# alexisvannson/GraphNet_Classifier

Measured on AMD Instinct MI355X. Metric: edges aggregated/sec (GraphNet forward), higher is better.
Workload: dtype f32; 1 GPU; c3: 1M nodes / 10M edges (6250 graphs x 160 nodes x 1600 edges), D=64, 2 GN blocks; graphs=6250, nodes=1000000, edges=10000000, n_blocks=2, width=64, step=CSR build + GraphNet.forward, inputs resident in HBM

## Files before the change

### graphnet_classifier_amd/csrc/mlp_device.h

```cpp
#pragma once
#include "gnc_common.h"

namespace gnc_mlp {

typedef float f32x16 __attribute__((ext_vector_type(16)));
typedef float f32x4 __attribute__((ext_vector_type(4)));

constexpr int KC = 64;
constexpr int LDSW = 68;
constexpr int RPW = 32;

__device__ __forceinline__ f32x16 mfma(float a, float b, f32x16 c) {
  return __builtin_amdgcn_mfma_f32_32x32x2f32(a, b, c, 0, 0, 0);
}

__device__ __forceinline__ void wave_lds_fence() {
  asm volatile("s_waitcnt lgkmcnt(0)" ::: "memory");
}

__device__ __forceinline__ float activate(float x, int act, float p) {
  switch (act) {
    case GNC_ACT_RELU: return x < 0.f ? 0.f : x;
    case GNC_ACT_IDENTITY: return x;
    case GNC_ACT_TANH: return tanhf(x);
    case GNC_ACT_SIGMOID: return 1.f / (1.f + expf(-x));
    case GNC_ACT_SILU: return x / (1.f + expf(-x));
    case GNC_ACT_GELU: return 0.5f * x * (1.f + erff(x * 0.70710678118654752440f));
    case GNC_ACT_LEAKY_RELU: return x < 0.f ? x * p : x;
    case GNC_ACT_ELU: return x > 0.f ? x : p * expm1f(x);
    default: return x;
  }
}

template <int T>
__device__ __forceinline__ void activate_tiles(f32x16 (&acc)[T], int act, float p) {
  if (act == GNC_ACT_RELU) {
#pragma unroll
    for (int t = 0; t < T; ++t)
#pragma unroll
      for (int r = 0; r < 16; ++r) acc[t][r] = acc[t][r] < 0.f ? 0.f : acc[t][r];
  } else {
#pragma unroll
    for (int t = 0; t < T; ++t)
#pragma unroll
      for (int r = 0; r < 16; ++r) acc[t][r] = activate(acc[t][r], act, p);
  }
}

__device__ __forceinline__ constexpr int feat_of(int t, int r, int h) { return 32 * t + (r & 3) + 8 * (r >> 2) + 4 * h; }

__device__ __forceinline__ f32x4 load4_guarded(const float* p, int col, int limit, bool vec_ok) {
  f32x4 v = {0.f, 0.f, 0.f, 0.f};
  if (vec_ok && col + 4 <= limit) {
    v = *reinterpret_cast<const f32x4*>(p);
  } else {
    if (col + 0 < limit) v.x = p[0];
    if (col + 1 < limit) v.y = p[1];
    if (col + 2 < limit) v.z = p[2];
    if (col + 3 < limit) v.w = p[3];
  }
  return v;
}

template <int TROWS, int NT>
__device__ __forceinline__ void stage_weights(float* wbuf, const float* __restrict__ W, int ldw, int out_dim,
                                              int kbase, int klimit, int ncol4, bool vec_ok, int tid) {
  constexpr int RPP = NT / 16;
  static_assert(TROWS % RPP == 0, "weight rows must be a multiple of the rows staged per pass");
  const int c4 = tid & 15;
  const int r0 = tid >> 4;
  if (c4 < ncol4) {
#pragma unroll
    for (int p = 0; p < TROWS / RPP; ++p) {
      const int n = p * RPP + r0;
      f32x4 v = {0.f, 0.f, 0.f, 0.f};
      if (n < out_dim) v = load4_guarded(W + (int64_t)n * ldw + kbase + c4 * 4, kbase + c4 * 4, klimit, vec_ok);
      *reinterpret_cast<f32x4*>(wbuf + n * LDSW + c4 * 4) = v;
    }
  }
}

template <int NT>
__device__ __forceinline__ void stage_params(float* pbuf, const gnc_mlp_desc_t& d, int pstride, int tid) {
  const int L = d.num_linear;
  const int out_dim = d.out_dim[L - 1];
  for (int idx = tid; idx < (L + 2) * pstride; idx += NT) {
    const int l = idx / pstride, n = idx - l * pstride;
    float v = 0.f;
    if (l < L) {
      if (d.bias[l] && n < d.out_dim[l]) v = d.bias[l][n];
    } else if (d.ln_gamma && n < out_dim) {
      v = (l == L) ? d.ln_gamma[n] : (d.ln_beta ? d.ln_beta[n] : 0.f);
    }
    pbuf[idx] = v;
  }
}

template <int T>
__device__ __forceinline__ void init_bias(f32x16 (&acc)[T], const float* pb, int h) {
#pragma unroll
  for (int t = 0; t < T; ++t)
#pragma unroll
    for (int q = 0; q < 4; ++q) {
      const f32x4 b = *reinterpret_cast<const f32x4*>(pb + 32 * t + 8 * q + 4 * h);
      acc[t][4 * q + 0] = b.x; acc[t][4 * q + 1] = b.y; acc[t][4 * q + 2] = b.z; acc[t][4 * q + 3] = b.w;
    }
}

template <int T>
__device__ __forceinline__ void mma_chunk_from_lds(f32x16 (&acc)[T], const float* abuf, const float* wbuf, int kc8,
                                                   int i, int h) {
#pragma unroll(T >= 4 ? 1 : 2)
  for (int g = 0; g < kc8; ++g) {
    const f32x4 b = *reinterpret_cast<const f32x4*>(abuf + i * LDSW + 8 * g + 4 * h);
#pragma unroll
    for (int t = 0; t < T; ++t) {
      const f32x4 a = *reinterpret_cast<const f32x4*>(wbuf + (32 * t + i) * LDSW + 8 * g + 4 * h);
      acc[t] = mfma(a.x, b.x, acc[t]);
      acc[t] = mfma(a.y, b.y, acc[t]);
      acc[t] = mfma(a.z, b.z, acc[t]);
      acc[t] = mfma(a.w, b.w, acc[t]);
    }
  }
}

template <int T>
__device__ __forceinline__ void add_rows_from_lds(f32x16 (&acc)[T], const float* abuf, int t0, int i, int h) {
#pragma unroll
  for (int tt = 0; tt < 2; ++tt) {
#pragma unroll
    for (int t = 0; t < T; ++t) {
      if (t == t0 + tt) {
#pragma unroll
        for (int q = 0; q < 4; ++q) {
          const f32x4 v = *reinterpret_cast<const f32x4*>(abuf + i * LDSW + 32 * tt + 8 * q + 4 * h);
          acc[t][4 * q + 0] += v.x; acc[t][4 * q + 1] += v.y; acc[t][4 * q + 2] += v.z; acc[t][4 * q + 3] += v.w;
        }
      }
    }
  }
}

template <int TI, int TO>
__device__ __forceinline__ void mma_chunk_from_regs(f32x16 (&dst)[TO], const f32x16 (&src)[TI], const float* wbuf,
                                                    int c, int in_dim, int i, int h) {
#pragma unroll
  for (int g = 0; g < 8; ++g) {
    const int ts = 2 * c + (g >> 2);
    if (ts < TI && c * KC + g * 8 < in_dim) {
      const int q = g & 3;
#pragma unroll
      for (int t = 0; t < TO; ++t) {
        const f32x4 a = *reinterpret_cast<const f32x4*>(wbuf + (32 * t + i) * LDSW + 8 * g + 4 * h);
        dst[t] = mfma(a.x, src[ts < TI ? ts : 0][4 * q + 0], dst[t]);
        dst[t] = mfma(a.y, src[ts < TI ? ts : 0][4 * q + 1], dst[t]);
        dst[t] = mfma(a.z, src[ts < TI ? ts : 0][4 * q + 2], dst[t]);
        dst[t] = mfma(a.w, src[ts < TI ? ts : 0][4 * q + 3], dst[t]);
      }
      if constexpr (TO >= 4) __builtin_amdgcn_sched_barrier(0);
    }
  }
}

typedef __bf16 bf16x8 __attribute__((ext_vector_type(8)));
typedef float f32x8 __attribute__((ext_vector_type(8)));

constexpr int SLDW = 72;
constexpr int SPLANE = 64 * SLDW;
constexpr int SCH = 3 * SPLANE / 2;

// ... 766 lines not shown
#pragma unroll
    for (int q = 0; q < 4; ++q) {
      f32x4 v = {o[TA][4 * q + 0], o[TA][4 * q + 1], o[TA][4 * q + 2], o[TA][4 * q + 3]};
      *reinterpret_cast<f32x4*>(abuf + i * LDSW + 32 * TT + 8 * q + 4 * h) = v;
    }
  }
}
template <int T, int T0>
__device__ __forceinline__ void chunk_to_lds(const f32x16 (&o)[T], float* abuf, int i, int h) {
  one_tile_to_lds<T, T0, 0>(o, abuf, i, h);
  one_tile_to_lds<T, T0 + 1, 1>(o, abuf, i, h);
}

struct SegView {
  const float* ptr;
  const int32_t* index;
  int ld;
  int width;
  uint32_t bytes;
};


struct BwdArgs {
  const float* grad_out;
  int ld_grad_out;
  float* act[GNC_MAX_LINEAR];
  float* dz[GNC_MAX_LINEAR];
  float* dx;
  int ld_dx;
  float* yhat;
  int dx_add_grad_out;
  float* ln_partial;
  const float* gg;
  const int* gg_index;
  int ld_gg;
  int64_t gg_rows;
  float* g_sum;
  int ld_g_sum;
};

__host__ __device__ inline int ldw_of(const gnc_mlp_desc_t& d, int l) { return d.ld_weight[l] ? d.ld_weight[l] : d.in_dim[l]; }

inline bool al16(const void* p) { return (reinterpret_cast<uintptr_t>(p) & 15u) == 0; }

inline int tiles_for(int width) {
  const int t = (width + 31) / 32;
  return t <= 1 ? 1 : t <= 2 ? 2 : t <= 4 ? 4 : 8;
}

int validate_desc(const gnc_mlp_desc_t* d, bool check_ptrs);
int launch_resident_dual(const float* x, int64_t ld_x, int64_t rows, const float* wa, int64_t ld_wa, const float* wb, int64_t ld_wb,
                         int in_dim, int out_dim, float* out_a, float* out_b, int64_t ld_out, hipStream_t stream, bool* launched);
int launch_resident(const gnc_mlp_desc_t& d, int T, bool narrow_out, hipStream_t stream, bool* launched,
                    bool probe_only = false, bool agg_only = false);
int launch_stream(const gnc_mlp_desc_t& d, int T, bool narrow_out, hipStream_t stream, bool* launched,
                  bool probe_only = false);
int launch_stream16(const gnc_mlp_desc_t& d, hipStream_t stream, bool* launched, bool probe_only = false);
int launch_col16(const gnc_mlp_desc_t& d, hipStream_t stream, bool* launched, bool probe_only = false);
int64_t col16_max_rows();
int64_t bwd_col16_max_rows();
bool bwd_col16_supported(const gnc_mlp_desc_t& d);
int bwd_col16_ln_partial_rows(int64_t rows);
int launch_bwd_col16(const gnc_mlp_bwd_desc_t& bd, hipStream_t stream);
bool bwd_col16_persist_supported(const gnc_mlp_desc_t& d);
int bwd_col16_persist_ln_partial_rows(int64_t rows);
int launch_bwd_col16_persist(const gnc_mlp_bwd_desc_t& bd, hipStream_t stream);
bool bwd_stream16_supported(const gnc_mlp_desc_t& d, bool want_dx);
int bwd_stream16_ln_partial_rows(int64_t rows);
int launch_bwd_stream16(const gnc_mlp_desc_t& d, const BwdArgs& b, hipStream_t stream, bool saved = false);

}
```

### graphnet_classifier_amd/csrc/mlp_fused.hip

```cpp
#include <stdlib.h>

#include "mlp_device.h"

using namespace gnc_mlp;

namespace {

constexpr int WAVES = 4;
constexpr int NT = WAVES * 64;
constexpr int RPB = RPW * WAVES;

__device__ __forceinline__ void stage_rows(float* abuf, const gnc_mlp_segment_t& seg, int64_t row0, int64_t rows,
                                           int c0, int ncol4, bool vec_ok, int lane) {
  const int c4 = lane & 15;
  const int rs = lane >> 4;
  if (c4 < ncol4) {
#pragma unroll
    for (int p = 0; p < RPW / 4; ++p) {
      const int j = p * 4 + rs;
      const int64_t r = row0 + j;
      f32x4 v = {0.f, 0.f, 0.f, 0.f};
      if (r < rows) {
        const int64_t tr = seg.index ? (int64_t)seg.index[r] : r;
        if (!seg.index || (uint64_t)tr < (uint64_t)seg.table_rows)
// ... 375 lines not shown
    gnc::set_error("gnc_mlp_operands_in_place_supported: this description runs on a kernel that reads rows of 16-B pieces");
    return GNC_ERR_UNSUPPORTED;
  }
  return GNC_OK;
}

extern "C" int gnc_mlp_edge_features_supported(const gnc_mlp_desc_t* desc) {
  int rc = validate_desc(desc, false);
  if (rc) return rc;
  const auto [T, narrow_out] = tile_class(*desc);
  gnc_mlp_desc_t probe = *desc;
  alignas(16) static float dummy_f[4];
  static int32_t dummy_i[1];
  if (!probe.ef_pos) probe.ef_pos = dummy_f;
  if (!probe.ef_src) probe.ef_src = dummy_i;
  if (!probe.ef_dst) probe.ef_dst = dummy_i;
  bool ok = false;
  {
    gnc_mlp_desc_t plain = *desc;
    plain.ef_pos = nullptr;
    if (!plain.seg[0].ptr) plain.seg[0].ptr = dummy_f;
    bool small = false;
    rc = launch_col16(plain, nullptr, &small, true);
    if (rc) return rc;
    if (!small && desc->rows > 0) {
      rc = launch_resident(probe, T, narrow_out, nullptr, &ok, true);
      if (rc) return rc;
    }
  }
  if (!ok) {
    gnc::set_error("gnc_mlp_edge_features_supported: needs the edge encoder's shape on the weights-resident kernel (one computed "
                   "segment of width 3 = space_dim 2, >= 2 Linear layers of widths 33..64, ReLU, no residual / save_act / agg_out) "
                   "and a batch above the small-batch limit");
    return GNC_ERR_UNSUPPORTED;
  }
  return GNC_OK;
}

extern "C" int gnc_mlp_small_batch_supported(const gnc_mlp_desc_t* desc) {
  int rc = validate_desc(desc, false);
  if (rc) return rc;
  FwdKernel k = FwdKernel::none;
  if (desc->rows > 0) {
    rc = forward_chain(*desc, nullptr, true, &k);
    if (rc) return rc;
  }
  if (k != FwdKernel::col16) {
    gnc::set_error("gnc_mlp_small_batch_supported: not a small-batch description (rows, widths <= 128, ReLU)");
    return GNC_ERR_UNSUPPORTED;
  }
  return GNC_OK;
}

extern "C" int gnc_mlp_forward_f32(const gnc_mlp_desc_t* desc, void* stream_) {
  int rc = validate_desc(desc, true);
  if (rc) return rc;
  if (desc->rows == 0) return GNC_OK;
  hipStream_t stream = (hipStream_t)stream_;
  if (desc->ef_pos) {
    rc = gnc_mlp_edge_features_supported(desc);
    if (rc) return rc;
    const auto [T, narrow_out] = tile_class(*desc);
    bool launched = false;
    rc = launch_resident(*desc, T, narrow_out, stream, &launched);
    if (!rc && !launched) {
      gnc::set_error("gnc_mlp_forward_f32: ef_pos given but the weights-resident kernel did not take the launch");
      rc = GNC_ERR_UNSUPPORTED;
    }
    return rc;
  }
  FwdKernel k;
  return forward_chain(*desc, stream, false, &k);
}
```

### graphnet_classifier_amd/csrc/mlp_resident.hip

```cpp
#include <stdlib.h>

#include "mlp_device.h"

using namespace gnc_mlp;

#ifdef GNC_PHASE_PROBE
__device__ unsigned long long gnc_phase_probe[4096 * 12];
extern "C" int gnc_phase_probe_read(void* dst, size_t bytes) {
  return (int)hipMemcpyFromSymbol(dst, HIP_SYMBOL(gnc_phase_probe), bytes);
}
#define PROBE_BEGIN() unsigned long long pr_acc[8] = {0, 0, 0, 0, 0, 0, 0, 0}, pr_tp, pr_tn; \
  const unsigned long long pr_c0 = __builtin_readcyclecounter(), pr_w0 = wall_clock64()
#define PROBE_TILE() pr_tp = __builtin_readcyclecounter()
#define PROBE(k) do { pr_tn = __builtin_readcyclecounter(); pr_acc[k] += pr_tn - pr_tp; pr_tp = pr_tn; } while (0)
#define PROBE_END() do { if ((threadIdx.x & 63) == 0) {                                                      \
    unsigned long long* o = gnc_phase_probe + (blockIdx.x * (blockDim.x >> 6) + (threadIdx.x >> 6)) * 12;    \
    for (int k = 0; k < 8; ++k) o[k] = pr_acc[k];                                                            \
    o[8] = __builtin_readcyclecounter() - pr_c0; o[9] = wall_clock64() - pr_w0; } } while (0)
#else
#define PROBE_BEGIN() do {} while (0)
#define PROBE_TILE() do {} while (0)
#define PROBE(k) do {} while (0)
#define PROBE_END() do {} while (0)
#endif

namespace {

constexpr int RWAVES = 8;
constexpr int RNT = RWAVES * 64;

template <int HT, int OT, int NMM, int NADD, bool RESREG, bool AGG = false, bool SAVE = false, bool FULL = false, int EF = 0, bool DUAL = false,
          int SPLIT = 0, bool AGGONLY = false>
__global__ __launch_bounds__(RNT) void mlp_resident_kernel(const gnc_mlp_desc_t d, const int num_wtiles,
                                                           const int total_chunks) {
  extern __shared__ __attribute__((aligned(16))) float lds[];
  constexpr int WT = HT > OT ? HT : OT;
  constexpr int CH = WT * 32 * LDSW;
  static_assert(!FULL || OT == 2, "fixed widths: 64 out");
  static_assert(!FULL || NADD == 2 || (NMM == 1 && !RESREG && !AGG && !SAVE && !DUAL), "fixed-width plain stacks");
  constexpr int SEGW = EF != 0 ? 3 : KC;
  constexpr bool W32 = FULL && !SAVE;
  constexpr bool GADD = W32 && NADD == 2;
  static_assert(SPLIT == 0 || (HT == 2 && SPLIT == 1 && NMM == 1 && ((NADD == 2 && RESREG && !DUAL) || (NADD == 0 && !RESREG))) ||
                    (HT == 2 && OT == 2 && SPLIT == 2 && NADD == 0 && !DUAL),
                "split shapes");
  constexpr int nf32 = SPLIT == 1 ? 0 : NMM;
  constexpr bool SPK = !(SPLIT == 1 && NADD == 2 && AGG && !FULL && !SAVE);
  constexpr bool PIPE = SPLIT != 0 && SPK && !DUAL && (FULL || (SPLIT == 2 && NMM == 1) || (SPLIT == 1 && NADD == 0));
  constexpr bool FRONT = GADD && SPLIT == 1 && PIPE;
  constexpr int GPK = FRONT ? 4 : 2;
  __bf16* const wsp = reinterpret_cast<__bf16*>(lds + nf32 * CH);
  auto wsplit = [&](int chunk) -> const __bf16* { return wsp + (chunk - nf32) * 3 * SPLANE; };
  constexpr int PSTRIDE = WT * 32;
  constexpr int NS = NMM + NADD;
  const int tid = threadIdx.x;
  const int lane = tid & 63;
  const int wave = __builtin_amdgcn_readfirstlane(tid >> 6);
  const int i = lane & 31;
  const int h = lane >> 5;
  const int c4 = lane & 15;
  const int rs = lane >> 4;
  const int L = FULL ? 3 : d.num_linear;
  const int out_dim = FULL ? KC : d.out_dim[L - 1];
  const int rows = (int)d.rows;
  float* wres = lds;
  float* pbuf = SPLIT == 0 ? lds + total_chunks * CH : lds + nf32 * CH + (total_chunks - nf32) * SCH;
  float* abuf = pbuf + (L + 2) * PSTRIDE + wave * RPW * LDSW;

  stage_params<RNT>(pbuf, d, PSTRIDE, tid);
  if constexpr (SPLIT != 0) {
    const int ldw0 = ldw_of(d, 0);
    const bool w0v = (ldw0 % 4 == 0) && ((reinterpret_cast<uintptr_t>(d.weight[0]) & 15u) == 0);
    if constexpr (SPLIT == 1) {
      stage_weights_split<RNT>(wsp, d.weight[0], ldw0, d.out_dim[0], d.seg[0].wcol, d.seg[0].wcol + d.seg[0].width,
                               w0v && (d.seg[0].wcol % 4 == 0), tid);
    } else {
#pragma unroll
      for (int s = 0; s < NMM; ++s)
        stage_weights<WT * 32, RNT>(wres + s * CH, d.weight[0], ldw0, d.out_dim[0], d.seg[s].wcol, d.seg[s].wcol + d.seg[s].width, 16,
                                    w0v && (d.seg[s].wcol % 4 == 0), tid);
    }
    if constexpr (DUAL) {
      const int ldw1 = ldw_of(d, 1);
      const bool w1v = (ldw1 % 4 == 0) && ((reinterpret_cast<uintptr_t>(d.weight[1]) & 15u) == 0) && (d.seg[0].wcol % 4 == 0);
      stage_weights_split<RNT>(wsp + 3 * SPLANE, d.weight[1], ldw1, d.out_dim[0], d.seg[0].wcol, d.seg[0].wcol + d.seg[0].width, w1v, tid);
    }
    for (int l = 1; l < L; ++l) {
      const int ldw = ldw_of(d, l);
      const bool wv = (ldw % 4 == 0) && ((reinterpret_cast<uintptr_t>(d.weight[l]) & 15u) == 0);
      stage_weights_split<RNT>(wsp + (NMM + l - 1 - nf32) * 3 * SPLANE, d.weight[l], ldw, d.out_dim[l], 0, d.in_dim[l], wv, tid);
    }
  } else {
    int chunk = 0;
    const int ldw0 = ldw_of(d, 0);
    const bool w0v = (ldw0 % 4 == 0) && ((reinterpret_cast<uintptr_t>(d.weight[0]) & 15u) == 0);
#pragma unroll
    for (int s = 0; s < NMM; ++s, ++chunk)
      stage_weights<WT * 32, RNT>(wres + chunk * CH, d.weight[0], ldw0, d.out_dim[0], d.seg[s].wcol,
                                  d.seg[s].wcol + d.seg[s].width, 16, w0v && (d.seg[s].wcol % 4 == 0), tid);
    for (int l = 1; l < L; ++l) {
      const int ldw = ldw_of(d, l);
      const bool wv = (ldw % 4 == 0) && ((reinterpret_cast<uintptr_t>(d.weight[l]) & 15u) == 0);
      for (int c = 0; c * KC < d.in_dim[l]; ++c, ++chunk)
        stage_weights<WT * 32, RNT>(wres + chunk * CH, d.weight[l], ldw, d.out_dim[l], c * KC, d.in_dim[l], 16, wv, tid);
    }
    if constexpr (DUAL) {
      const int ldw1 = ldw_of(d, 1);
      const bool w1v = (ldw1 % 4 == 0) && ((reinterpret_cast<uintptr_t>(d.weight[1]) & 15u) == 0);
      stage_weights<WT * 32, RNT>(wres + CH, d.weight[1], ldw1, d.out_dim[0], d.seg[0].wcol, d.seg[0].wcol + d.seg[0].width, 16,
                                  w1v && (d.seg[0].wcol % 4 == 0), tid);
    }
  }
  __syncthreads();

  SegView sv[NS];
#pragma unroll
  for (int s = 0; s < NS; ++s) sv[s] = {d.seg[s].ptr, (W32 && RESREG && s == NMM - 1) ? nullptr : d.seg[s].index, d.seg[s].ld, FULL ? SEGW : d.seg[s].width,
                                          (uint32_t)(d.seg[s].table_rows * d.seg[s].ld * 4)};
  if constexpr (GADD) {
    __builtin_assume(sv[NMM].index != nullptr);
    __builtin_assume(sv[NMM + 1].index != nullptr);
  }

  const int total_waves = (int)gridDim.x * RWAVES;
  const int last_wt = num_wtiles - 1;

  auto row_offset = [&](int wt, const SegView& s) -> uint32_t {
    if (s.index == nullptr) return 0;
    const int wtc = wt < last_wt ? wt : last_wt;
    int r = wtc * RPW + (lane & 31);
    r = r < rows ? r : rows - 1;
    return (uint32_t)s.index[r];
  };
  auto load_rows = [&](f32x4 (&pre)[NP], const SegView& s, int wt, uint32_t off) {
    const int col = c4 * 4 < s.ld ? c4 * 4 : 0;
    if (s.index == nullptr) {
      if constexpr (W32)
        load_tile_rows_w(pre, table_window(s.ptr, rows, s.ld), s.ld, (wt < num_wtiles ? wt : num_wtiles) * RPW, rows, (uint32_t)(rs * s.ld + col) * 4u);
      else load_tile_rows(pre, s.ptr, s.ld, (int64_t)wt * RPW, rows, (uint32_t)(rs * s.ld + col) * 4u);
    } else {
      const __amdgpu_buffer_rsrc_t w = __builtin_amdgcn_make_buffer_rsrc(const_cast<float*>(s.ptr), 0, (int)s.bytes, 0x00020000);
      const uint32_t row_bytes = off * (uint32_t)(s.ld * 4);
#pragma unroll
      for (int p = 0; p < NP; ++p) pre[p] = window_load(w, (uint32_t)__shfl((int)row_bytes, p * 4 + rs, 64) + (uint32_t)(col * 4));
    }
  };
  auto stage = [&](const f32x4 (&pre)[NP], int width) {
    compiler_lds_barrier();
    const int c = c4 * 4;
    if (width >= KC) {
#pragma unroll
      for (int p = 0; p < NP; ++p) *reinterpret_cast<f32x4*>(abuf + (p * 4 + rs) * LDSW + c) = pre[p];
    } else {
#pragma unroll
      for (int p = 0; p < NP; ++p) {
        f32x4 v = pre[p];
        v.x = c + 0 < width ? v.x : 0.f; v.y = c + 1 < width ? v.y : 0.f;
        v.z = c + 2 < width ? v.z : 0.f; v.w = c + 3 < width ? v.w : 0.f;
        *reinterpret_cast<f32x4*>(abuf + (p * 4 + rs) * LDSW + c) = v;
      }
    }
    compiler_lds_barrier();
  };

  const int gwave = (int)blockIdx.x * RWAVES + wave;
  const int stride = AGG ? 1 : total_waves;
  int wt = gwave, wt_end = num_wtiles;
  if constexpr (AGG) {
    const int q = num_wtiles / total_waves, rem = num_wtiles - q * total_waves;
    wt = gwave * q + (gwave < rem ? gwave : rem);
    wt_end = wt + q + (gwave < rem ? 1 : 0);
  }
  f32x4 cur[NP];
  f32x4 addA[NADD ? NP : 1], addB[NADD ? NP : 1];
  uint32_t offs[NS];
  typedef float f32x2 __attribute__((ext_vector_type(2)));
  int ef_s = 0, ef_d = 0;
  f32x2 ef_ps = {0.f, 0.f}, ef_pd = {0.f, 0.f};
  const __amdgpu_buffer_rsrc_t ef_win =
      __builtin_amdgcn_make_buffer_rsrc(const_cast<float*>(EF == 1 ? d.ef_pos : nullptr), 0, EF == 1 ? (int)(uint32_t)(d.ef_nodes * 8) : 0, 0x00020000);
  auto ef_ids = [&](int t) {
    const int tc = t < last_wt ? t : last_wt;
    int r = tc * RPW + (lane & 31);
    r = r < rows ? r : rows - 1;
    ef_s = d.ef_src[r];
    ef_d = d.ef_dst[r];
  };
  auto ef_fetch = [&]() {
    typedef uint32_t u32x2 __attribute__((ext_vector_type(2)));
    ef_ps = __builtin_bit_cast(f32x2, (u32x2)__builtin_amdgcn_raw_buffer_load_b64(ef_win, (uint32_t)ef_s * 8u, 0, 0));
    ef_pd = __builtin_bit_cast(f32x2, (u32x2)__builtin_amdgcn_raw_buffer_load_b64(ef_win, (uint32_t)ef_d * 8u, 0, 0));
  };
  auto ef_stage = [&]() {
    compiler_lds_barrier();
    const float dx = ef_pd.x - ef_ps.x, dy = ef_pd.y - ef_ps.y;
    f32x4 v = {dx, dy, __builtin_fabsf(dx) + __builtin_fabsf(dy), 0.f};
    if (h) v = f32x4{0.f, 0.f, 0.f, 0.f};
    *reinterpret_cast<f32x4*>(abuf + i * LDSW + 4 * h) = v;
    compiler_lds_barrier();
  };
  typedef float f32x3 __attribute__((ext_vector_type(3)));
  f32x3 n3_row = {0.f, 0.f, 0.f};
  const __amdgpu_buffer_rsrc_t n3_win = __builtin_amdgcn_make_buffer_rsrc(
      const_cast<float*>(EF == 2 ? d.seg[0].ptr : nullptr), 0, EF == 2 ? (int)(uint32_t)(d.rows * 12) : 0, 0x00020000);
  auto n3_fetch = [&](int t) {
    typedef uint32_t u32x3 __attribute__((ext_vector_type(3)));
    const int tc = t < last_wt ? t : last_wt;
    n3_row = __builtin_bit_cast(f32x3, (u32x3)__builtin_amdgcn_raw_buffer_load_b96(n3_win, (uint32_t)(tc * RPW + (lane & 31)) * 12u, 0, 0));
  };
  auto n3_stage = [&]() {
    compiler_lds_barrier();
    f32x4 v = {n3_row.x, n3_row.y, n3_row.z, 0.f};
    if (h) v = f32x4{0.f, 0.f, 0.f, 0.f};
    *reinterpret_cast<f32x4*>(abuf + i * LDSW + 4 * h) = v;
    compiler_lds_barrier();
  };
  uint32_t off0 = 0;
  if constexpr (EF == 1) {
// ... 106 lines not shown
                  mma_group_split<HT>(hid, split_lds_group<SPK>(abuf, kg, i, h), wch, kg, i, h);
                  request(kg);
                }
              }
            } else {
            const float* wch = wres + s * CH;
#pragma unroll
            for (int g = 0; g < 8; ++g) {
              const f32x4 b = *reinterpret_cast<const f32x4*>(abuf + i * LDSW + 8 * g + 4 * h);
#pragma unroll
              for (int t = 0; t < HT; ++t) {
                const f32x4 a = *reinterpret_cast<const f32x4*>(wch + (32 * t + i) * LDSW + 8 * g + 4 * h);
                hid[t] = mfma(a.x, b.x, hid[t]);
                hid[t] = mfma(a.y, b.y, hid[t]);
                hid[t] = mfma(a.z, b.z, hid[t]);
                hid[t] = mfma(a.w, b.w, hid[t]);
              }
              const uint32_t oa = (uint32_t)na + cola, ob = (uint32_t)nb + colb;
              if (g + 1 < 8) {
                na = __shfl(rba, (g + 1) * 4 + rs, 64);
                nb = __shfl(rbb, (g + 1) * 4 + rs, 64);
              }
              addA[g] = window_load(wa, oa);
              addB[g] = window_load(wb, ob);
            }
            }
            offs[NMM] = row_offset(nwt, sv[NMM]);
            offs[NMM + 1] = row_offset(nwt, sv[NMM + 1]);
            interleaved = true;
          } else {
            load_rows(addA, sv[NMM], wt, offs[NMM]);
            load_rows(addB, sv[NMM + 1], wt, offs[NMM + 1]);
            offs[NMM] = row_offset(nwt, sv[NMM]);
            offs[NMM + 1] = row_offset(nwt, sv[NMM + 1]);
          }
        } else if constexpr (EF == 1) {
          ef_fetch();
          ef_ids(nwt + stride);
        } else if constexpr (EF == 2) {
          n3_fetch(nwt);
        } else {
          load_rows(cur, sv[0], nwt, off0);
          off0 = row_offset(nwt + stride, sv[0]);
        }
      }
      PROBE(7);
      if (!interleaved) {
        if constexpr (SPLIT == 1 && DUAL) {}
        else if constexpr (SPLIT == 1) {
          const int kc16 = (sv[s].width + 15) >> 4;
          if (PIPE && kc16 == 4 && L > 1) mma_chunk_from_lds_split_pipe<HT, 4>(hid, abuf, wsplit(s), i, h);
          else mma_chunk_from_lds_split<HT, SPK>(hid, abuf, wsplit(s), kc16, i, h);
        }
        else mma_chunk_from_lds<HT>(hid, abuf, wres + s * CH, (sv[s].width + 7) >> 3, i, h);
      }
      if constexpr (RESREG && !FRONT) if (s == NMM - 1) {
#pragma unroll
        for (int t = 0; t < HT; ++t)
#pragma unroll
          for (int q = 0; q < 4; ++q) {
            const f32x4 v = *reinterpret_cast<const f32x4*>(abuf + i * LDSW + 32 * t + 8 * q + 4 * h);
            res[t][4 * q + 0] = v.x; res[t][4 * q + 1] = v.y; res[t][4 * q + 2] = v.z; res[t][4 * q + 3] = v.w;
          }
      }
      PROBE(1);
    }
    if constexpr (NADD > 0) {
      if constexpr (!FRONT) {
        f32x4 sum[NP];
#pragma unroll
        for (int p = 0; p < NP; ++p) sum[p] = addA[p] + addB[p];
        stage(sum, sv[NMM].width);
      }
      load_rows(cur, sv[0], nwt, off0);
      off0 = row_offset(nwt + stride, sv[0]);
      add_tile_from_lds<HT>(hid, abuf, i, h);
      PROBE(2);
    }

    f32x16 hidb[DUAL ? HT : 1];
    if constexpr (DUAL) {
      init_bias<HT>(hidb, pbuf, h);
      if constexpr (SPLIT == 1) {
        const int kc16 = (sv[0].width + 15) >> 4;
#pragma unroll
        for (int kg = 0; kg < 4; ++kg)
          if (kg < kc16) {
            const bf16x8x3 x = split_lds_group(abuf, kg, i, h);
            mma_group_split<HT>(hid, x, wsplit(0), kg, i, h);
            mma_group_split<HT>(hidb, x, wsplit(1), kg, i, h);
          }
      } else {
        mma_chunk_from_lds<HT>(hidb, abuf, wres + CH, (sv[0].width + 7) >> 3, i, h);
      }
    }
    if (L == 1) {
      if (d.ln_gamma) layer_norm_tiles<HT>(hid, pbuf + L * PSTRIDE, pbuf + (L + 1) * PSTRIDE, out_dim, d.ln_eps, h);
      if constexpr (RESREG) {
#pragma unroll
        for (int t = 0; t < HT; ++t) hid[t] += res[t];
      }
      compiler_lds_barrier();
      tiles_to_lds<HT>(hid, abuf, i, h);
    } else {
      if constexpr (SPLIT == 0) relu_tiles_fmaxf<HT>(hid);
      else relu_tiles<HT, NADD ? 0 : SPLIT == 1 ? MFMA_STATES_BF16_32X32X16 : MFMA_STATES_F32_32X32X2>(hid);
      auto save_rows = [&](const f32x16 (&acc)[HT], int l) {
// ... 113 lines not shown
        if (col_out < out_dim) {
          if (row0 + RPW <= rows) {
            uint32_t r0b;
            const __amdgpu_buffer_rsrc_t ow = full_tile_window(d.out, row0, rows, d.ld_out, &r0b);
#pragma unroll
            for (int p = 0; p < NP; ++p) hidden_window_store_s<true>(outv[p], out_lane_off + r0b, ow, (uint32_t)(p * 16 * d.ld_out));
          } else {
#pragma unroll
            for (int p = 0; p < NP; ++p) hidden_window_store(outv[p], out_lane_off, row_window(d.out, row0 + 4 * p, rows, d.ld_out));
          }
        }
      } else {
#pragma unroll
        for (int p = 0; p < NP; ++p) {
          const int r = row0 + p * 4 + rs;
          store_row_piece(d.out + (int64_t)(r < rows ? r : rows - 1) * d.ld_out, col_out, outv[p], r < rows && col_out < out_dim,
                          out_dim, false);
        }
      }
    }
    if constexpr (DUAL) {
      compiler_lds_barrier();
      tiles_to_lds<HT>(hidb, abuf, i, h);
      compiler_lds_barrier();
      f32x4 outb[NP];
#pragma unroll
      for (int p = 0; p < NP; ++p) outb[p] = *reinterpret_cast<const f32x4*>(abuf + (p * 4 + rs) * LDSW + col_out);
      if (col_out < out_dim) {
        if (row0 + RPW <= rows) {
          uint32_t r0b;
          const __amdgpu_buffer_rsrc_t ow = full_tile_window(d.save_act[0], row0, rows, d.ld_out, &r0b);
#pragma unroll
          for (int p = 0; p < NP; ++p) hidden_window_store_s<true>(outb[p], out_lane_off + r0b, ow, (uint32_t)(p * 16 * d.ld_out));
        } else {
#pragma unroll
          for (int p = 0; p < NP; ++p) hidden_window_store(outb[p], out_lane_off, row_window(d.save_act[0], row0 + 4 * p, rows, d.ld_out));
        }
      }
    }
    compiler_lds_barrier();
    PROBE(6);
    wt = nwt;
  }
  if constexpr (AGG) {
    if (lane == 0) {
      d.agg_fix[2 * gwave] = agg_first ? agg_cur : agg_first_dst;
      d.agg_fix[2 * gwave + 1] = agg_cur;
    }
  }
  PROBE_END();
}

template <int HT, int OT, int NMM, int NADD, bool RESREG, bool AGG = false, bool SAVE = false, bool FULL = false, int EF = 0, bool DUAL = false,
          int SPLIT = 0, bool AGGONLY = false>
int launch(const gnc_mlp_desc_t& d, int total_chunks, size_t smem, hipStream_t stream) {
  void (*const kernel)(const gnc_mlp_desc_t, const int, const int) = &mlp_resident_kernel<HT, OT, NMM, NADD, RESREG, AGG, SAVE, FULL, EF, DUAL, SPLIT, AGGONLY>;
  static bool attr_set = false;
  if (!attr_set) {
    int rc = gnc::check_hip(hipFuncSetAttribute(reinterpret_cast<const void*>(kernel), hipFuncAttributeMaxDynamicSharedMemorySize, 160 * 1024),
                            "hipFuncSetAttribute(MaxDynamicSharedMemorySize)");
    if (rc) return rc;
    attr_set = true;
  }
  const int64_t num_wtiles = gnc::ceil_div(d.rows, RPW);
  int64_t grid = gnc::ceil_div(num_wtiles, RWAVES);
  if (grid > gnc::num_cu()) grid = gnc::num_cu();
  if constexpr (AGG) grid = gnc::num_cu();
  kernel<<<dim3((unsigned)grid), dim3(RNT), smem, stream>>>(d, (int)num_wtiles, total_chunks);
  return gnc::check_launch("mlp_resident_kernel");
}

template <int HT, int OT, int NMM, int NADD, bool RESREG, bool AGG = false, bool SAVE = false, bool FULL = false, int EF = 0,
          bool AGGONLY = false>
int launch_cls(int split, const gnc_mlp_desc_t& d, int total_chunks, size_t smem, hipStream_t stream) {
  if constexpr (HT == 2 && OT == 2 && NMM == 1 && NADD == 2 && RESREG) {
    if (split == 1) return launch<HT, OT, NMM, NADD, RESREG, AGG, SAVE, FULL, EF, false, 1, AGGONLY>(d, total_chunks, smem, stream);
  }
  if constexpr (HT == 2 && NMM == 1 && NADD == 0 && !RESREG && !AGG && !SAVE && !FULL && EF == 0) {
    if (split == 1) return launch<HT, OT, NMM, NADD, RESREG, AGG, SAVE, FULL, EF, false, 1>(d, total_chunks, smem, stream);
  }
  if constexpr (HT == 2 && OT == 2 && NADD == 0 && !AGG && (!FULL || EF != 0) && ((NMM == 1 && !RESREG) || (NMM == 2 && EF == 0))) {
    if (split == 2) return launch<HT, OT, NMM, NADD, RESREG, AGG, SAVE, FULL, EF, false, 2>(d, total_chunks, smem, stream);
  }
  if (split) return GNC_ERR_UNSUPPORTED;
  return launch<HT, OT, NMM, NADD, RESREG, AGG, SAVE, FULL, EF, false, 0, AGGONLY>(d, total_chunks, smem, stream);
}

}

static bool f32_exact() {
  static const bool v = getenv("GNC_MLP_F32_EXACT") != nullptr;
  return v;
}

extern "C" int gnc_mlp_agg_fix_len(void) { return 2 * gnc::num_cu() * RWAVES; }

int gnc_mlp::launch_resident_dual(const float* x, int64_t ld_x, int64_t rows, const float* wa, int64_t ld_wa, const float* wb,
                                  int64_t ld_wb, int in_dim, int out_dim, float* out_a, float* out_b, int64_t ld_out,
                                  hipStream_t stream, bool* launched) {
  *launched = false;
  static const bool disabled = getenv("GNC_MLP_NO_RESIDENT") != nullptr;
  if (disabled || rows < 1 || rows >= INT32_MAX || in_dim < 1 || in_dim > KC || out_dim <= 32 || out_dim > KC || out_dim % 4 != 0 ||
      ld_x % 4 != 0 || ld_x < in_dim || ld_out % 4 != 0 || ld_out < out_dim || ld_wa < in_dim || ld_wb < in_dim || ld_wa > INT32_MAX ||
      ld_wb > INT32_MAX || ld_x > INT32_MAX || ld_out > INT32_MAX || !al16(x) || !al16(out_a) || !al16(out_b))
    return GNC_OK;
  gnc_mlp_desc_t d = {};
  d.num_segments = 1;
  d.num_linear = 1;
  d.activation = GNC_ACT_RELU;
  d.seg[0].ptr = x;
  d.seg[0].width = in_dim;
  d.seg[0].ld = (int32_t)ld_x;
  d.seg[0].mode = GNC_SEG_MATMUL;
  d.weight[0] = wa;
  d.ld_weight[0] = (int32_t)ld_wa;
  d.weight[1] = wb;
  d.ld_weight[1] = (int32_t)ld_wb;
  d.in_dim[0] = in_dim;
  d.out_dim[0] = out_dim;
  d.in_dim[1] = in_dim;
  d.out = out_a;
  d.save_act[0] = out_b;
  d.ld_out = (int32_t)ld_out;
  d.rows = rows;
  const int total_chunks = 2;
  const bool split = !f32_exact();
  const size_t floats = (size_t)total_chunks * (split ? SCH : 2 * 32 * LDSW) + (size_t)(1 + 2) * 2 * 32 + (size_t)RWAVES * RPW * LDSW;
  *launched = true;
  return split ? launch<2, 2, 1, 0, false, false, false, false, 0, true, 1>(d, total_chunks, floats * sizeof(float), stream)
               : launch<2, 2, 1, 0, false, false, false, false, 0, true>(d, total_chunks, floats * sizeof(float), stream);
}

int gnc_mlp::launch_resident(const gnc_mlp_desc_t& d, int T, bool narrow_out, hipStream_t stream, bool* launched,
                             bool probe_only, bool agg_only) {
  *launched = false;
  if (agg_only && (!d.agg_out || d.save_act[0])) return GNC_OK;
  static const bool disabled = getenv("GNC_MLP_NO_RESIDENT") != nullptr;
  if (disabled) return GNC_OK;
  if (T > 2 || d.rows >= INT32_MAX) return GNC_OK;
  const int L = d.num_linear;
  const int od = d.out_dim[L - 1];
  if (L > 1 && d.activation != GNC_ACT_RELU) return GNC_OK;
  int nmm = 0, nadd = 0;
  bool n3 = false;
  for (int s = 0; s < d.num_segments; ++s) {
    const gnc_mlp_segment_t& g = d.seg[s];
    if (d.ef_pos && s == 0) continue;
    if (s == 0 && d.num_segments == 1 && !g.index && g.mode == GNC_SEG_MATMUL && g.width == 3 && g.ld == 3 &&
        (reinterpret_cast<uintptr_t>(g.ptr) & 3u) == 0 && d.rows * 12 <= 0xffffffffll && !d.residual && !d.save_act[0] && !d.agg_out &&
        !narrow_out && L >= 2 && T == 2) {
      n3 = true;
      ++nmm;
      continue;
    }
    if (g.width > KC || g.ld % 4 != 0 || !al16(g.ptr)) return GNC_OK;
    if (g.index && (g.table_rows <= 0 || g.table_rows * (int64_t)g.ld * 4 > 0xffffffffll)) return GNC_OK;
    if (g.mode == GNC_SEG_ADD) {
      ++nadd;
    } else {
      if (nadd) return GNC_OK;
      ++nmm;
    }
  }
  if (d.ef_pos) {
    ++nmm;
    const gnc_mlp_segment_t& g = d.seg[0];
    if (d.num_segments != 1 || g.mode != GNC_SEG_MATMUL || g.index || d.ef_space_dim != 2 || g.width != 3 || !d.ef_src || !d.ef_dst ||
        d.ef_nodes <= 0 || d.ef_nodes * 8 > 0xffffffffll || d.residual || d.save_act[0] || d.agg_out || narrow_out || L < 2 || T != 2)
      return GNC_OK;
  }
  if (nmm < 1 || nmm > 3 || (nadd != 0 && !(nadd == 2 && nmm == 1))) return GNC_OK;
  if (d.residual && (d.ld_residual % 4 != 0 || !al16(d.residual))) return GNC_OK;
  if (L > 1 && d.in_dim[1] > KC) return GNC_OK;
  if (d.save_act[0]) {
    if (L < 2) return GNC_OK;
    for (int l = 0; l < L - 1; ++l)
      if (!d.save_act[l] || d.out_dim[l] % 4 != 0 || !al16(d.save_act[l])) return GNC_OK;
  }

  const int total_chunks = nmm + (L - 1);
  const gnc_mlp_segment_t& lm = d.seg[nmm - 1];
  const bool resreg = d.residual && d.residual == lm.ptr && !lm.index && lm.ld == d.ld_residual && lm.width == od;

  int split = 0;
  if (!f32_exact() && T == 2) {
    bool hidden64 = true, row_ordered = !d.ef_pos && !n3;
    for (int l = 0; l < L - 1; ++l) hidden64 = hidden64 && d.out_dim[l] == KC;
    for (int s = 0; s < d.num_segments; ++s) row_ordered = row_ordered && !d.seg[s].index;
    if (nadd == 2) {
      if (nmm == 1 && resreg && L >= 2 && !narrow_out) split = 1;
    } else if (nmm == 1 && !resreg && row_ordered && (L == 1 ? !narrow_out : (narrow_out && hidden64))) {
      split = 1;
    } else if (L >= 2 && !narrow_out && hidden64) {
      if (nmm == 1 && !resreg && d.seg[0].width <= 4) split = 2;
      else if (nmm == 2 && row_ordered) split = 2;
    }
  }
  auto smem_of = [&](int nsplit) {
    return ((size_t)(total_chunks - nsplit) * T * 32 * LDSW + (size_t)nsplit * SCH + (size_t)(L + 2) * T * 32 +
            (size_t)RWAVES * RPW * LDSW) * sizeof(float);
  };
  if (split && smem_of(split == 1 ? total_chunks : total_chunks - nmm) > 160 * 1024) split = 0;
  const size_t smem = smem_of(split == 1 ? total_chunks : (split == 2 ? total_chunks - nmm : 0));
  if (smem > 160 * 1024) return GNC_OK;

  if (narrow_out && (resreg || nadd || nmm != 1)) return GNC_OK;
  static const bool no_full = getenv("GNC_MLP_NO_FULL64") != nullptr;
  bool full64 = !no_full && L == 3 && od == KC && d.ln_gamma && d.ld_out % 4 == 0 && al16(d.out);
  for (int s = 0; s < d.num_segments; ++s) full64 = full64 && (d.seg[s].width == KC || d.ef_pos || n3);
  for (int l = 0; l < L; ++l) full64 = full64 && d.out_dim[l] == KC && (l == 0 || d.in_dim[l] == KC);
  auto fits32 = [&](int64_t ld) { return (d.rows + 2 * RPW) * ld * 4 <= 0xffffffffll; };
  bool win32 = fits32(d.ld_out);
  for (int s = 0; s < d.num_segments; ++s) {
    const gnc_mlp_segment_t& g = d.seg[s];
    if (!g.index && !(s == 0 && (d.ef_pos || n3))) win32 = win32 && fits32(g.ld);
    if (g.mode == GNC_SEG_ADD && !g.index) win32 = false;
  }
  const bool full32 = full64 && win32;
  const bool plain64 = full32 && T == 2 && nmm == 1 && nadd == 0 && !d.residual;
  if (d.ef_pos) {
    *launched = true;
    if (probe_only) return GNC_OK;
    if (plain64) return launch_cls<2, 2, 1, 0, false, false, false, true, 1>(split, d, total_chunks, smem, stream);
    return launch_cls<2, 2, 1, 0, false, false, false, false, 1>(split, d, total_chunks, smem, stream);
  }
  if (n3) {
    *launched = true;
    if (probe_only) return GNC_OK;
    if (plain64) return launch_cls<2, 2, 1, 0, false, false, false, true, 2>(split, d, total_chunks, smem, stream);
    return launch_cls<2, 2, 1, 0, false, false, false, false, 2>(split, d, total_chunks, smem, stream);
  }
  if (d.save_act[0]) {
    if (T != 2 || narrow_out || nmm > 2 || L < 2) return GNC_OK;
    if (nmm == 2 && (nadd != 0 || d.agg_out)) return GNC_OK;
    if (d.agg_out && !(nadd == 2 && resreg && d.agg_index && d.agg_fix && d.ld_agg >= od)) return GNC_OK;
    if (nadd == 2 && !resreg) return GNC_OK;
    *launched = true;
    if (probe_only) return GNC_OK;
    if (nmm == 2)
      return resreg ? launch_cls<2, 2, 2, 0, true, false, true>(split, d, total_chunks, smem, stream)
                    : launch_cls<2, 2, 2, 0, false, false, true>(split, d, total_chunks, smem, stream);
    if (d.agg_out) return full64 ? launch_cls<2, 2, 1, 2, true, true, true, true>(split, d, total_chunks, smem, stream)
                                 : launch_cls<2, 2, 1, 2, true, true, true>(split, d, total_chunks, smem, stream);
    if (nadd == 2) return launch_cls<2, 2, 1, 2, true, false, true>(split, d, total_chunks, smem, stream);
    return resreg ? launch<2, 2, 1, 0, true, false, true>(d, total_chunks, smem, stream)
                  : launch_cls<2, 2, 1, 0, false, false, true>(split, d, total_chunks, smem, stream);
  }
  if (d.agg_out) {
    if (!(nadd == 2 && nmm == 1 && resreg && !narrow_out && d.agg_index && d.agg_fix && d.ld_agg >= od)) return GNC_OK;
    if (agg_only && !(T == 2 && full32)) return GNC_OK;
    *launched = true;
    if (probe_only) return GNC_OK;
    if (agg_only) return launch_cls<2, 2, 1, 2, true, true, false, true, 0, true>(split, d, total_chunks, smem, stream);
    if (T == 2 && full32) return launch_cls<2, 2, 1, 2, true, true, false, true>(split, d, total_chunks, smem, stream);
    return T == 2 ? launch_cls<2, 2, 1, 2, true, true>(split, d, total_chunks, smem, stream)
                  : launch<1, 1, 1, 2, true, true>(d, total_chunks, smem, stream);
  }
  if (probe_only) {
    *launched = true;
    return GNC_OK;
  }
#define GNC_RES(HT_, NMM_, NADD_)                                                             \
  do {                                                                                        \
    *launched = true;                                                                         \
    return resreg ? launch<HT_, HT_, NMM_, NADD_, true>(d, total_chunks, smem, stream)        \
                  : launch<HT_, HT_, NMM_, NADD_, false>(d, total_chunks, smem, stream);      \
  } while (0)
  if (narrow_out) {
    *launched = true;
    return T == 2 ? launch_cls<2, 1, 1, 0, false>(split, d, total_chunks, smem, stream)
                  : launch<1, 1, 1, 0, false>(d, total_chunks, smem, stream);
  }
  if (T == 2) {
    *launched = true;
    if (nadd == 2) return resreg ? launch_cls<2, 2, 1, 2, true>(split, d, total_chunks, smem, stream)
// ... 15 lines not shown
```

Before: 3.637 billion edges/s.

## Run edge-feature encoder with 12 waves per block using compact first-layer weights

Adds a 12-wave variant of the resident MLP kernel for the fixed-width edge-position encoder (split=2, 3-wide input). The first-layer weight chunk is stored with an 8-float LDS stride instead of 68, which frees enough shared memory for four more per-wave row buffers within the 160KB limit. Weight staging now adapts its rows-per-pass to the thread count. The aim is more waves per CU to hide memory latency in the edge encoder. The cost is more register and LDS pressure per CU and a new kernel instantiation that needs validating.

```diff
diff --git a/graphnet_classifier_amd/csrc/mlp_device.h b/graphnet_classifier_amd/csrc/mlp_device.h
--- a/graphnet_classifier_amd/csrc/mlp_device.h
+++ b/graphnet_classifier_amd/csrc/mlp_device.h
@@ -62,20 +62,27 @@
   return v;
 }
 
-template <int TROWS, int NT>
+constexpr int stage_rows_per_pass(int trows, int nt) {
+  int r = nt / 16;
+  while (trows % r) --r;
+  return r;
+}
+
+constexpr int LDSW1 = 8;
+
+template <int TROWS, int NT, int LDW = LDSW>
 __device__ __forceinline__ void stage_weights(float* wbuf, const float* __restrict__ W, int ldw, int out_dim,
                                               int kbase, int klimit, int ncol4, bool vec_ok, int tid) {
-  constexpr int RPP = NT / 16;
-  static_assert(TROWS % RPP == 0, "weight rows must be a multiple of the rows staged per pass");
+  constexpr int RPP = stage_rows_per_pass(TROWS, NT);
   const int c4 = tid & 15;
   const int r0 = tid >> 4;
-  if (c4 < ncol4) {
+  if (c4 < ncol4 && (RPP * 16 == NT || r0 < RPP)) {
 #pragma unroll
     for (int p = 0; p < TROWS / RPP; ++p) {
       const int n = p * RPP + r0;
       f32x4 v = {0.f, 0.f, 0.f, 0.f};
       if (n < out_dim) v = load4_guarded(W + (int64_t)n * ldw + kbase + c4 * 4, kbase + c4 * 4, klimit, vec_ok);
-      *reinterpret_cast<f32x4*>(wbuf + n * LDSW + c4 * 4) = v;
+      *reinterpret_cast<f32x4*>(wbuf + n * LDW + c4 * 4) = v;
     }
   }
 }
@@ -107,7 +114,7 @@
     }
 }
 
-template <int T>
+template <int T, int LDW = LDSW>
 __device__ __forceinline__ void mma_chunk_from_lds(f32x16 (&acc)[T], const float* abuf, const float* wbuf, int kc8,
                                                    int i, int h) {
 #pragma unroll(T >= 4 ? 1 : 2)
@@ -115,7 +122,7 @@
     const f32x4 b = *reinterpret_cast<const f32x4*>(abuf + i * LDSW + 8 * g + 4 * h);
 #pragma unroll
     for (int t = 0; t < T; ++t) {
-      const f32x4 a = *reinterpret_cast<const f32x4*>(wbuf + (32 * t + i) * LDSW + 8 * g + 4 * h);
+      const f32x4 a = *reinterpret_cast<const f32x4*>(wbuf + (32 * t + i) * LDW + 8 * g + 4 * h);
       acc[t] = mfma(a.x, b.x, acc[t]);
       acc[t] = mfma(a.y, b.y, acc[t]);
       acc[t] = mfma(a.z, b.z, acc[t]);
@@ -988,7 +995,10 @@
 int launch_resident_dual(const float* x, int64_t ld_x, int64_t rows, const float* wa, int64_t ld_wa, const float* wb, int64_t ld_wb,
                          int in_dim, int out_dim, float* out_a, float* out_b, int64_t ld_out, hipStream_t stream, bool* launched);
 int launch_resident(const gnc_mlp_desc_t& d, int T, bool narrow_out, hipStream_t stream, bool* launched,
-                    bool probe_only = false, bool agg_only = false);
+                    bool probe_only = false, bool agg_only = false, int* waves = nullptr);
+constexpr size_t RESIDENT_LDS_LIMIT = 160 * 1024;
+size_t resident_lds_bytes(int fp32_chunks, int split_chunks, int L, int T, int waves, bool compact_first);
+int encoder_waves(int fp32_chunks, int split_chunks, int L, int T);
 int launch_stream(const gnc_mlp_desc_t& d, int T, bool narrow_out, hipStream_t stream, bool* launched,
                   bool probe_only = false);
 int launch_stream16(const gnc_mlp_desc_t& d, hipStream_t stream, bool* launched, bool probe_only = false);
diff --git a/graphnet_classifier_amd/csrc/mlp_fused.hip b/graphnet_classifier_amd/csrc/mlp_fused.hip
--- a/graphnet_classifier_amd/csrc/mlp_fused.hip
+++ b/graphnet_classifier_amd/csrc/mlp_fused.hip
@@ -451,6 +451,21 @@
   return GNC_OK;
 }
 
+extern "C" int gnc_mlp_resident_waves(const gnc_mlp_desc_t* desc) {
+  if (validate_desc(desc, false) || desc->rows <= 0) return 0;
+  if (desc->ef_pos) {
+    if (gnc_mlp_edge_features_supported(desc)) return 0;
+  } else {
+    FwdKernel k = FwdKernel::none;
+    if (forward_chain(*desc, nullptr, true, &k) || k != FwdKernel::resident) return 0;
+  }
+  const auto [T, narrow_out] = tile_class(*desc);
+  bool ok = false;
+  int waves = 0;
+  if (launch_resident(*desc, T, narrow_out, nullptr, &ok, true, false, &waves) || !ok) return 0;
+  return waves;
+}
+
 extern "C" int gnc_mlp_forward_f32(const gnc_mlp_desc_t* desc, void* stream_) {
   int rc = validate_desc(desc, true);
   if (rc) return rc;
diff --git a/graphnet_classifier_amd/csrc/mlp_resident.hip b/graphnet_classifier_amd/csrc/mlp_resident.hip
--- a/graphnet_classifier_amd/csrc/mlp_resident.hip
+++ b/graphnet_classifier_amd/csrc/mlp_resident.hip
@@ -28,14 +28,20 @@
 
 constexpr int RWAVES = 8;
 constexpr int RNT = RWAVES * 64;
+constexpr int RWAVES12 = 12;
 
 template <int HT, int OT, int NMM, int NADD, bool RESREG, bool AGG = false, bool SAVE = false, bool FULL = false, int EF = 0, bool DUAL = false,
-          int SPLIT = 0, bool AGGONLY = false>
-__global__ __launch_bounds__(RNT) void mlp_resident_kernel(const gnc_mlp_desc_t d, const int num_wtiles,
-                                                           const int total_chunks) {
+          int SPLIT = 0, bool AGGONLY = false, int WAVES = RWAVES>
+__global__ __launch_bounds__(WAVES * 64) void mlp_resident_kernel(const gnc_mlp_desc_t d, const int num_wtiles,
+                                                                  const int total_chunks) {
   extern __shared__ __attribute__((aligned(16))) float lds[];
   constexpr int WT = HT > OT ? HT : OT;
   constexpr int CH = WT * 32 * LDSW;
+  constexpr int NT_ = WAVES * 64;
+  constexpr bool W12 = WAVES == RWAVES12;
+  static_assert(WAVES == RWAVES || (W12 && FULL && EF == 1 && SPLIT == 2 && NMM == 1), "three waves per SIMD: the class-2 fixed-width edge encoder");
+  constexpr int LDW0 = W12 ? LDSW1 : LDSW;
+  constexpr int CH0 = WT * 32 * LDW0;
   static_assert(!FULL || OT == 2, "fixed widths: 64 out");
   static_assert(!FULL || NADD == 2 || (NMM == 1 && !RESREG && !AGG && !SAVE && !DUAL), "fixed-width plain stacks");
   constexpr int SEGW = EF != 0 ? 3 : KC;
@@ -49,7 +55,7 @@
   constexpr bool PIPE = SPLIT != 0 && SPK && !DUAL && (FULL || (SPLIT == 2 && NMM == 1) || (SPLIT == 1 && NADD == 0));
   constexpr bool FRONT = GADD && SPLIT == 1 && PIPE;
   constexpr int GPK = FRONT ? 4 : 2;
-  __bf16* const wsp = reinterpret_cast<__bf16*>(lds + nf32 * CH);
+  __bf16* const wsp = reinterpret_cast<__bf16*>(lds + nf32 * CH0);
   auto wsplit = [&](int chunk) -> const __bf16* { return wsp + (chunk - nf32) * 3 * SPLANE; };
   constexpr int PSTRIDE = WT * 32;
   constexpr int NS = NMM + NADD;
@@ -64,31 +70,31 @@
   const int out_dim = FULL ? KC : d.out_dim[L - 1];
   const int rows = (int)d.rows;
   float* wres = lds;
-  float* pbuf = SPLIT == 0 ? lds + total_chunks * CH : lds + nf32 * CH + (total_chunks - nf32) * SCH;
+  float* pbuf = SPLIT == 0 ? lds + total_chunks * CH : lds + nf32 * CH0 + (total_chunks - nf32) * SCH;
   float* abuf = pbuf + (L + 2) * PSTRIDE + wave * RPW * LDSW;
 
-  stage_params<RNT>(pbuf, d, PSTRIDE, tid);
+  stage_params<NT_>(pbuf, d, PSTRIDE, tid);
   if constexpr (SPLIT != 0) {
     const int ldw0 = ldw_of(d, 0);
     const bool w0v = (ldw0 % 4 == 0) && ((reinterpret_cast<uintptr_t>(d.weight[0]) & 15u) == 0);
     if constexpr (SPLIT == 1) {
-      stage_weights_split<RNT>(wsp, d.weight[0], ldw0, d.out_dim[0], d.seg[0].wcol, d.seg[0].wcol + d.seg[0].width,
+      stage_weights_split<NT_>(wsp, d.weight[0], ldw0, d.out_dim[0], d.seg[0].wcol, d.seg[0].wcol + d.seg[0].width,
                                w0v && (d.seg[0].wcol % 4 == 0), tid);
     } else {
 #pragma unroll
       for (int s = 0; s < NMM; ++s)
-        stage_weights<WT * 32, RNT>(wres + s * CH, d.weight[0], ldw0, d.out_dim[0], d.seg[s].wcol, d.seg[s].wcol + d.seg[s].width, 16,
-                                    w0v && (d.seg[s].wcol % 4 == 0), tid);
+        stage_weights<WT * 32, NT_, LDW0>(wres + s * CH0, d.weight[0], ldw0, d.out_dim[0], d.seg[s].wcol, d.seg[s].wcol + d.seg[s].width,
+                                          W12 ? LDSW1 / 4 : 16, w0v && (d.seg[s].wcol % 4 == 0), tid);
     }
     if constexpr (DUAL) {
       const int ldw1 = ldw_of(d, 1);
       const bool w1v = (ldw1 % 4 == 0) && ((reinterpret_cast<uintptr_t>(d.weight[1]) & 15u) == 0) && (d.seg[0].wcol % 4 == 0);
-      stage_weights_split<RNT>(wsp + 3 * SPLANE, d.weight[1], ldw1, d.out_dim[0], d.seg[0].wcol, d.seg[0].wcol + d.seg[0].width, w1v, tid);
+      stage_weights_split<NT_>(wsp + 3 * SPLANE, d.weight[1], ldw1, d.out_dim[0], d.seg[0].wcol, d.seg[0].wcol + d.seg[0].width, w1v, tid);
     }
     for (int l = 1; l < L; ++l) {
       const int ldw = ldw_of(d, l);
       const bool wv = (ldw % 4 == 0) && ((reinterpret_cast<uintptr_t>(d.weight[l]) & 15u) == 0);
-      stage_weights_split<RNT>(wsp + (NMM + l - 1 - nf32) * 3 * SPLANE, d.weight[l], ldw, d.out_dim[l], 0, d.in_dim[l], wv, tid);
+      stage_weights_split<NT_>(wsp + (NMM + l - 1 - nf32) * 3 * SPLANE, d.weight[l], ldw, d.out_dim[l], 0, d.in_dim[l], wv, tid);
     }
   } else {
     int chunk = 0;
@@ -96,18 +102,18 @@
     const bool w0v = (ldw0 % 4 == 0) && ((reinterpret_cast<uintptr_t>(d.weight[0]) & 15u) == 0);
 #pragma unroll
     for (int s = 0; s < NMM; ++s, ++chunk)
-      stage_weights<WT * 32, RNT>(wres + chunk * CH, d.weight[0], ldw0, d.out_dim[0], d.seg[s].wcol,
+      stage_weights<WT * 32, NT_>(wres + chunk * CH, d.weight[0], ldw0, d.out_dim[0], d.seg[s].wcol,
                                   d.seg[s].wcol + d.seg[s].width, 16, w0v && (d.seg[s].wcol % 4 == 0), tid);
     for (int l = 1; l < L; ++l) {
       const int ldw = ldw_of(d, l);
       const bool wv = (ldw % 4 == 0) && ((reinterpret_cast<uintptr_t>(d.weight[l]) & 15u) == 0);
       for (int c = 0; c * KC < d.in_dim[l]; ++c, ++chunk)
-        stage_weights<WT * 32, RNT>(wres + chunk * CH, d.weight[l], ldw, d.out_dim[l], c * KC, d.in_dim[l], 16, wv, tid);
+        stage_weights<WT * 32, NT_>(wres + chunk * CH, d.weight[l], ldw, d.out_dim[l], c * KC, d.in_dim[l], 16, wv, tid);
     }
     if constexpr (DUAL) {
       const int ldw1 = ldw_of(d, 1);
       const bool w1v = (ldw1 % 4 == 0) && ((reinterpret_cast<uintptr_t>(d.weight[1]) & 15u) == 0);
-      stage_weights<WT * 32, RNT>(wres + CH, d.weight[1], ldw1, d.out_dim[0], d.seg[0].wcol, d.seg[0].wcol + d.seg[0].width, 16,
+      stage_weights<WT * 32, NT_>(wres + CH, d.weight[1], ldw1, d.out_dim[0], d.seg[0].wcol, d.seg[0].wcol + d.seg[0].width, 16,
                                   w1v && (d.seg[0].wcol % 4 == 0), tid);
     }
   }
@@ -122,7 +128,7 @@
     __builtin_assume(sv[NMM + 1].index != nullptr);
   }
 
-  const int total_waves = (int)gridDim.x * RWAVES;
+  const int total_waves = (int)gridDim.x * WAVES;
   const int last_wt = num_wtiles - 1;
 
   auto row_offset = [&](int wt, const SegView& s) -> uint32_t {
@@ -163,7 +169,7 @@
     compiler_lds_barrier();
   };
 
-  const int gwave = (int)blockIdx.x * RWAVES + wave;
+  const int gwave = (int)blockIdx.x * WAVES + wave;
   const int stride = AGG ? 1 : total_waves;
   int wt = gwave, wt_end = num_wtiles;
   if constexpr (AGG) {
@@ -376,7 +382,7 @@
           if (PIPE && kc16 == 4 && L > 1) mma_chunk_from_lds_split_pipe<HT, 4>(hid, abuf, wsplit(s), i, h);
           else mma_chunk_from_lds_split<HT, SPK>(hid, abuf, wsplit(s), kc16, i, h);
         }
-        else mma_chunk_from_lds<HT>(hid, abuf, wres + s * CH, (sv[s].width + 7) >> 3, i, h);
+        else mma_chunk_from_lds<HT, LDW0>(hid, abuf, wres + s * CH0, (sv[s].width + 7) >> 3, i, h);
       }
       if constexpr (RESREG && !FRONT) if (s == NMM - 1) {
 #pragma unroll
@@ -596,9 +602,9 @@
 }
 
 template <int HT, int OT, int NMM, int NADD, bool RESREG, bool AGG = false, bool SAVE = false, bool FULL = false, int EF = 0, bool DUAL = false,
-          int SPLIT = 0, bool AGGONLY = false>
+          int SPLIT = 0, bool AGGONLY = false, int WAVES = RWAVES>
 int launch(const gnc_mlp_desc_t& d, int total_chunks, size_t smem, hipStream_t stream) {
-  void (*const kernel)(const gnc_mlp_desc_t, const int, const int) = &mlp_resident_kernel<HT, OT, NMM, NADD, RESREG, AGG, SAVE, FULL, EF, DUAL, SPLIT, AGGONLY>;
+  void (*const kernel)(const gnc_mlp_desc_t, const int, const int) = &mlp_resident_kernel<HT, OT, NMM, NADD, RESREG, AGG, SAVE, FULL, EF, DUAL, SPLIT, AGGONLY, WAVES>;
   static bool attr_set = false;
   if (!attr_set) {
     int rc = gnc::check_hip(hipFuncSetAttribute(reinterpret_cast<const void*>(kernel), hipFuncAttributeMaxDynamicSharedMemorySize, 160 * 1024),
@@ -607,10 +613,10 @@
     attr_set = true;
   }
   const int64_t num_wtiles = gnc::ceil_div(d.rows, RPW);
-  int64_t grid = gnc::ceil_div(num_wtiles, RWAVES);
+  int64_t grid = gnc::ceil_div(num_wtiles, WAVES);
   if (grid > gnc::num_cu()) grid = gnc::num_cu();
   if constexpr (AGG) grid = gnc::num_cu();
-  kernel<<<dim3((unsigned)grid), dim3(RNT), smem, stream>>>(d, (int)num_wtiles, total_chunks);
+  kernel<<<dim3((unsigned)grid), dim3(WAVES * 64), smem, stream>>>(d, (int)num_wtiles, total_chunks);
   return gnc::check_launch("mlp_resident_kernel");
 }
 
@@ -675,9 +681,27 @@
                : launch<2, 2, 1, 0, false, false, false, false, 0, true>(d, total_chunks, floats * sizeof(float), stream);
 }
 
+size_t gnc_mlp::resident_lds_bytes(int fp32_chunks, int split_chunks, int L, int T, int waves, bool compact_first) {
+  const int compact = compact_first && fp32_chunks > 0 ? 1 : 0;
+  return ((size_t)compact * T * 32 * LDSW1 + (size_t)(fp32_chunks - compact) * T * 32 * LDSW + (size_t)split_chunks * SCH +
+          (size_t)(L + 2) * T * 32 + (size_t)waves * RPW * LDSW) * sizeof(float);
+}
+
+int gnc_mlp::encoder_waves(int fp32_chunks, int split_chunks, int L, int T) {
+  return resident_lds_bytes(fp32_chunks, split_chunks, L, T, RWAVES12, true) <= RESIDENT_LDS_LIMIT ? RWAVES12 : RWAVES;
+}
+
+extern "C" int64_t gnc_mlp_resident_lds_bytes(int fp32_chunks, int split_chunks, int num_linear, int tiles, int waves, int compact_first) {
+  return (int64_t)gnc_mlp::resident_lds_bytes(fp32_chunks, split_chunks, num_linear, tiles, waves, compact_first != 0);
+}
+extern "C" int gnc_mlp_encoder_waves(int fp32_chunks, int split_chunks, int num_linear, int tiles) {
+  return gnc_mlp::encoder_waves(fp32_chunks, split_chunks, num_linear, tiles);
+}
+
 int gnc_mlp::launch_resident(const gnc_mlp_desc_t& d, int T, bool narrow_out, hipStream_t stream, bool* launched,
-                             bool probe_only, bool agg_only) {
+                             bool probe_only, bool agg_only, int* waves) {
   *launched = false;
+  if (waves) *waves = 0;
   if (agg_only && (!d.agg_out || d.save_act[0])) return GNC_OK;
   static const bool disabled = getenv("GNC_MLP_NO_RESIDENT") != nullptr;
   if (disabled) return GNC_OK;
@@ -741,12 +765,11 @@
     }
   }
   auto smem_of = [&](int nsplit) {
-    return ((size_t)(total_chunks - nsplit) * T * 32 * LDSW + (size_t)nsplit * SCH + (size_t)(L + 2) * T * 32 +
-            (size_t)RWAVES * RPW * LDSW) * sizeof(float);
-  };
-  if (split && smem_of(split == 1 ? total_chunks : total_chunks - nmm) > 160 * 1024) split = 0;
-  const size_t smem = smem_of(split == 1 ? total_chunks : (split == 2 ? total_chunks - nmm : 0));
-  if (smem > 160 * 1024) return GNC_OK;
+    return resident_lds_bytes(total_chunks - nsplit, nsplit, L, T, RWAVES, false);
+  };
+  if (split && smem_of(split == 1 ? total_chunks : total_chunks - nmm) > RESIDENT_LDS_LIMIT) split = 0;
+  size_t smem = smem_of(split == 1 ? total_chunks : (split == 2 ? total_chunks - nmm : 0));
+  if (smem > RESIDENT_LDS_LIMIT) return GNC_OK;
 
   if (narrow_out && (resreg || nadd || nmm != 1)) return GNC_OK;
   static const bool no_full = getenv("GNC_MLP_NO_FULL64") != nullptr;
@@ -762,9 +785,14 @@
   }
   const bool full32 = full64 && win32;
   const bool plain64 = full32 && T == 2 && nmm == 1 && nadd == 0 && !d.residual;
+  static const bool no_waves12 = getenv("GNC_MLP_NO_WAVES12") != nullptr;
+  const bool waves12 = !no_waves12 && plain64 && split == 2 && d.ef_pos && encoder_waves(nmm, total_chunks - nmm, L, T) == RWAVES12;
+  if (waves12) smem = resident_lds_bytes(nmm, total_chunks - nmm, L, T, RWAVES12, true);
+  if (waves) *waves = waves12 ? RWAVES12 : RWAVES;
   if (d.ef_pos) {
     *launched = true;
     if (probe_only) return GNC_OK;
+    if (waves12) return launch<2, 2, 1, 0, false, false, false, true, 1, false, 2, false, RWAVES12>(d, total_chunks, smem, stream);
     if (plain64) return launch_cls<2, 2, 1, 0, false, false, false, true, 1>(split, d, total_chunks, smem, stream);
     return launch_cls<2, 2, 1, 0, false, false, false, false, 1>(split, d, total_chunks, smem, stream);
   }
```

Result: no change. 3.653 billion edges/s, median of 6 (+0.5%).
